# byronknoll/gmix

Measured on AMD Instinct MI355X. Metric: mixer bits/sec (synthetic 256-input mixer streams, forward+update), higher is better.
Workload: dtype f32; 1 GPU; configs[1]: synthetic 256-input 1-layer mixer (1 mixer, 2^16-row gate table), random logits, forward+update; n_inputs=256, mixers=1/0/0, streams_per_gpu=4096, total_bits=5452595200, parallelism=streams sharded over 1 GPU(s), no collective on the data path

## Files before the change

gmix_amd/csrc/gmx_capi.cpp:

```cpp
#include <hip/hip_runtime.h>
#include <math.h>
#include <stddef.h>
#include <stdio.h>
#include <stdlib.h>
#include <string.h>
#include <time.h>

#include <algorithm>
#include <cmath>
#include <atomic>
#include <map>
#include <new>
#include <string>
#include <vector>

#include "../../include/gmxmix.h"
#include "../../include/gmxmix_lstm_group.h"
#include "../../include/gmxmix_decoder.h"
#include "../../include/gmxmix_lstm_shape.h"
#include "../../include/gmxmix_encoder.h"
#include "../../include/gmxmix_analysis.h"
#include "../../include/gmxmix_ppmd.h"
#include "gmx_buildhash.h"
#include "gmx_internal.h"
// ... 1088 lines not shown
  a.seed = seed ? seed : 0x9E3779B97F4A7C15ull;
  a.n = t.n;
  a.n_pad = t.n_pad;
  a.m = t.m;
  a.mask_words = t.mask_words;
  a.n_streams = b->S;
  a.restart = restart ? 1 : 0;
  a.ctx_mode = ctx_mode;
  a.bit_mode = bit_mode;
  a.ctx_mod = ctx_mod;
  a.zero_mod = zero_mod;
  HIPCHK(gmx_launch_synth_kernel(&a, b->g->stream));
  return batch_note_device_use(b);
}

extern "C" int gmx_group_run(gmx_group* g, gmx_batch* b, uint64_t n_bits, int learn, float* kernel_ms) {
  if (!g || !b || b->g != g || b->S != g->S || n_bits > b->max_bits) return GMX_ERR_INVALID;
  HIPCHK(hipSetDevice(g->device));
  int rc = sessions_close(g, false);
  if (rc) return rc;
  std::fill(g->fwd_done.begin(), g->fwd_done.end(), 0);
  return launch_run(g, b, 0, 0, g->S, n_bits, GMX_MODE_PREDICT | (learn ? GMX_MODE_LEARN : 0u),
                    kernel_ms);
}

extern "C" int gmx_group_run_ragged(gmx_group* g, gmx_batch* b, const uint64_t* n_bits, int learn) {
  if (!g || !b || b->g != g || b->S != g->S || !n_bits) return GMX_ERR_INVALID;
  uint64_t maxn = 0;
  bool same = true;
  for (int s = 0; s < g->S; ++s) {
    if (n_bits[s] > b->max_bits) return GMX_ERR_INVALID;
    maxn = std::max(maxn, n_bits[s]);
    same = same && n_bits[s] == n_bits[0];
  }
  HIPCHK(hipSetDevice(g->device));
  int rc = sessions_close(g, false);
  if (rc) return rc;
  std::fill(g->fwd_done.begin(), g->fwd_done.end(), 0);
  const unsigned mode = GMX_MODE_PREDICT | (learn ? GMX_MODE_LEARN : 0u);
  if (same) return launch_run(g, b, 0, 0, g->S, maxn, mode, nullptr);
  const GmxKernelKind kind = kernel_for(g, mode);
  static const bool split = getenv("GMX_RAGGED_SPLIT") != nullptr;
  if (!split && (kind == GMX_K_STOCK || kind == GMX_K_BANK || kind == GMX_K_PAIR)) return launch_run(g, b, 0, 0, g->S, maxn, mode, nullptr, n_bits);
  for (int s0 = 0; s0 < g->S;) {
    int s1 = s0 + 1;
    while (s1 < g->S && n_bits[s1] == n_bits[s0]) ++s1;
    rc = launch_run(g, b, s0, s0, s1 - s0, n_bits[s0], mode, nullptr);
    if (rc) return rc;
    s0 = s1;
  }
  return GMX_OK;
}

static int ensure_one(gmx_group* g) {
  if (g->one) return GMX_OK;
  int rc = batch_alloc(&g->one, g, g->S, 1, GMX_BATCH_OUTPUTS | GMX_BATCH_MASK);
  if (rc) return rc;
  if (!gmx_batch_predictions(g->one) || !gmx_batch_active_mask(g->one) || !gmx_batch_contexts(g->one) ||
      !gmx_batch_bits(g->one) || !gmx_batch_p(g->one) || !gmx_batch_outputs(g->one))
    return GMX_ERR_NOMEM;
  return GMX_OK;
}

extern "C" int gmx_bank_forward(gmx_group* g, int stream, const float* predictions,
                                const int32_t* active_models, int n_active, const uint32_t* contexts,
                                float* p_final, float* out_all) {
  if (!g || stream < 0 || stream >= g->S || !predictions || !contexts) return GMX_ERR_INVALID;
  if (n_active > 0 && !active_models) return GMX_ERR_INVALID;
  HIPCHK(hipSetDevice(g->device));
  int rc;
  if (g->use_sessions && group_is_stock(g)) {
    rc = session_forward(g, stream, predictions, active_models, n_active, contexts, p_final, out_all);
    if (rc == GMX_OK) g->fwd_done[stream] = 2;
    if (rc != GMX_ERR_STATE) return rc;
  }
  rc = sessions_close(g, true);
  if (rc) return rc;
  rc = ensure_one(g);
  if (rc) return rc;
  gmx_batch* b = g->one;
  const GmxTopoDev& t = g->topo;
  const size_t s = (size_t)stream;
  HIPCHK(hipStreamSynchronize(g->stream));
  float* hp = b->h_pred + s * t.n_pad;
  uint32_t* hm = b->h_mask + s * t.mask_words;
  uint32_t* hc = b->h_ctx + s * t.m;
  memcpy(hp, predictions, t.n * sizeof(float));
  for (int i = t.n; i < t.n_pad; ++i) hp[i] = 0.f;
  if (n_active < 0) {
    for (int w = 0; w < t.mask_words; ++w) hm[w] = 0xffffffffu;
  } else {
    for (int w = 0; w < t.mask_words; ++w) hm[w] = 0;
    for (int i = 0; i < n_active; ++i) {
      int idx = active_models[i];
      if (idx < 0 || idx >= t.n) return GMX_ERR_INVALID;
      hm[idx >> 5] |= 1u << (idx & 31);
    }
  }
  memcpy(hc, contexts, t.m * sizeof(uint32_t));
  HIPCHK(hipMemcpyAsync(b->d_pred + s * t.n_pad, hp, t.n_pad * 4, hipMemcpyHostToDevice, g->stream));
  HIPCHK(hipMemcpyAsync(b->d_mask + s * t.mask_words, hm, t.mask_words * 4, hipMemcpyHostToDevice,
                        g->stream));
  HIPCHK(hipMemcpyAsync(b->d_ctx + s * t.m, hc, t.m * 4, hipMemcpyHostToDevice, g->stream));
  rc = launch_run(g, b, stream, stream, 1, 1, GMX_MODE_PREDICT | GMX_MODE_LATCH, nullptr);
  if (rc) return rc;
  HIPCHK(hipMemcpyAsync(b->h_p + s, b->d_p + s, 4, hipMemcpyDeviceToHost, g->stream));
  if (out_all)
    HIPCHK(hipMemcpyAsync(b->h_out + s * t.m, b->d_out + s * t.m, t.m * 4, hipMemcpyDeviceToHost,
                          g->stream));
  HIPCHK(hipStreamSynchronize(g->stream));
  if (p_final) *p_final = b->h_p[s];
  if (out_all) memcpy(out_all, b->h_out + s * t.m, t.m * sizeof(float));
  g->fwd_done[stream] = 1;
  return GMX_OK;
}

extern "C" int gmx_bank_learn(gmx_group* g, int stream, int bit) {
  if (!g || stream < 0 || stream >= g->S || (bit != 0 && bit != 1)) return GMX_ERR_INVALID;
  if (!g->fwd_done[stream]) return GMX_ERR_STATE;
  HIPCHK(hipSetDevice(g->device));
  if (g->fwd_done[stream] == 2) {
    int rcs = session_learn(g, stream, bit);
    if (rcs == GMX_OK) g->fwd_done[stream] = 0;
    return rcs;
  }
  if (!g->one) return GMX_ERR_STATE;
  gmx_batch* b = g->one;
  HIPCHK(hipStreamSynchronize(g->stream));
  b->h_bits[stream] = (uint8_t)bit;
  HIPCHK(hipMemcpyAsync(b->d_bits + stream, b->h_bits + stream, 1, hipMemcpyHostToDevice, g->stream));
  int rc = launch_run(g, b, stream, stream, 1, 1, GMX_MODE_LEARN, nullptr);
  if (rc) return rc;
  HIPCHK(hipStreamSynchronize(g->stream));
  g->fwd_done[stream] = 0;
  return GMX_OK;
}

#include "gmx_lockstep.inc"

static int fetch_bank(gmx_group* g, int stream, std::vector<uint8_t>& img) {
  img.resize(g->topo.bank_bytes);
  HIPCHK(hipSetDevice(g->device));
  int rc = sessions_close(g, true);
  if (rc) return rc;
  HIPCHK(hipStreamSynchronize(g->stream));
  HIPCHK(hipMemcpy(img.data(), g->banks + (size_t)stream * g->topo.bank_bytes, img.size(),
                   hipMemcpyDeviceToHost));
  return GMX_OK;
}

extern "C" int gmx_bank_export(gmx_group* g, int stream, void* long_buf, size_t* long_bytes,
                               void* short_buf, size_t* short_bytes) {
  if (!g || stream < 0 || stream >= g->S || !long_bytes || !short_bytes) return GMX_ERR_INVALID;
  const GmxTopoDev& t = g->topo;
  std::vector<uint8_t> img;
  int rc = fetch_bank(g, stream, img);
  if (rc) return rc;
  const size_t need_short = (size_t)t.m * 24;
  size_t need_long = 0;
  for (int j = 0; j < t.m; ++j) {
    need_long += 8;
    for (uint32_t r = 0; r < t.mx[j].table_size; ++r)
      if (*GMX_RS_PTR(img.data(), t.mx[j], r)) need_long += 12 + 4 * (size_t)t.mx[j].weight_size;
  }
  const bool fits = long_buf && short_buf && *long_bytes >= need_long && *short_bytes >= need_short;
  *long_bytes = need_long;
  *short_bytes = need_short;
  if (!long_buf && !short_buf) return GMX_OK;
  if (!fits) return GMX_ERR_INVALID;
  memcpy(short_buf, img.data() + t.scal_off, need_short);
  uint8_t* o = (uint8_t*)long_buf;
  for (int j = 0; j < t.m; ++j) {
    const GmxMixerDev& x = t.mx[j];
    const float* w = (const float*)(img.data() + x.w_off);
    uint32_t cnt = 0;
    for (uint32_t r = 0; r < x.table_size; ++r)
      if (*GMX_RS_PTR(img.data(), x, r)) ++cnt;
    uint32_t input_size = cnt ? x.weight_size : 0;
    memcpy(o, &cnt, 4);
    memcpy(o + 4, &input_size, 4);
    o += 8;
    for (uint32_t r = 0; r < x.table_size; ++r) {
      const uint64_t steps = *GMX_RS_PTR(img.data(), x, r);
      if (!steps) continue;
      memcpy(o, &r, 4);
      memcpy(o + 4, &steps, 8);
      memcpy(o + 12, w + (size_t)r * x.stride, 4 * (size_t)x.weight_size);
      o += 12 + 4 * (size_t)x.weight_size;
    }
  }
  return GMX_OK;
}

extern "C" int gmx_bank_import(gmx_group* g, int stream, const void* long_buf, size_t long_bytes,
                               const void* short_buf, size_t short_bytes) {
  if (!g || stream < 0 || stream >= g->S || !long_buf || !short_buf) return GMX_ERR_INVALID;
  const GmxTopoDev& t = g->topo;
  if (short_bytes != (size_t)t.m * 24) return GMX_ERR_FORMAT;
  std::vector<uint8_t> img(t.bank_bytes, 0);
  memcpy(img.data() + t.scal_off, short_buf, short_bytes);
  const uint64_t* sc = (const uint64_t*)(img.data() + t.scal_off);
  for (int j = 1; j < t.m; ++j)
    if (sc[3 * j] != sc[0]) return GMX_ERR_FORMAT;
  const uint8_t* p = (const uint8_t*)long_buf;
  const uint8_t* end = p + long_bytes;
  for (int j = 0; j < t.m; ++j) {
    const GmxMixerDev& x = t.mx[j];
    if (end - p < 8) return GMX_ERR_FORMAT;
    uint32_t cnt, input_size;
    memcpy(&cnt, p, 4);
    memcpy(&input_size, p + 4, 4);
    p += 8;
    if (cnt > x.table_size || (cnt && input_size != x.weight_size)) return GMX_ERR_FORMAT;
    float* w = (float*)(img.data() + x.w_off);
    for (uint32_t i = 0; i < cnt; ++i) {
      if ((size_t)(end - p) < 12 + 4 * (size_t)input_size) return GMX_ERR_FORMAT;
      uint32_t r;
      memcpy(&r, p, 4);
      if (r >= x.table_size) return GMX_ERR_FORMAT;
      uint64_t* const rs = GMX_RS_PTR(img.data(), x, r);
      memcpy(rs, p + 4, 8);
      if (*rs == 0) return GMX_ERR_FORMAT;
      memcpy(w + (size_t)r * x.stride, p + 12, 4 * (size_t)input_size);
      p += 12 + 4 * (size_t)input_size;
    }
  }
  if (p != end) return GMX_ERR_FORMAT;
  HIPCHK(hipSetDevice(g->device));
  int rc = sessions_close(g, true);
  if (rc) return rc;
  if (stream < (int)g->sessions.size() && g->sessions[stream]) g->sessions[stream]->fwd_live = false;
  HIPCHK(hipStreamSynchronize(g->stream));
  HIPCHK(hipMemcpy(g->banks + (size_t)stream * t.bank_bytes, img.data(), img.size(),
                   hipMemcpyHostToDevice));
  g->steps[stream] = sc[0];
  g->fwd_done[stream] = 0;
  for (gmx_lockstep* ls : g->locksteps) ls->predicted = false;
  return GMX_OK;
}

extern "C" int gmx_bank_copy(gmx_group* dst, int dst_stream, gmx_group* src, int src_stream) {
  if (!dst || !src || dst_stream < 0 || dst_stream >= dst->S || src_stream < 0 || src_stream >= src->S)
    return GMX_ERR_INVALID;
  const GmxTopoDev &a = dst->topo, &b = src->topo;
  if (a.m != b.m || a.n != b.n || a.n_skip != b.n_skip || a.bank_bytes != b.bank_bytes)
    return GMX_ERR_INVALID;
  for (int j = 0; j < a.m; ++j)
    if (a.mx[j].table_size != b.mx[j].table_size || a.mx[j].weight_size != b.mx[j].weight_size ||
        a.mx[j].layer != b.mx[j].layer)
      return GMX_ERR_INVALID;
  HIPCHK(hipSetDevice(src->device));
  int rc = sessions_close(src, true);
  if (rc) return rc;
  HIPCHK(hipStreamSynchronize(src->stream));
  HIPCHK(hipSetDevice(dst->device));
  rc = sessions_close(dst, true);
  if (rc) return rc;
  if (dst_stream < (int)dst->sessions.size() && dst->sessions[dst_stream])
    dst->sessions[dst_stream]->fwd_live = false;
  HIPCHK(hipStreamSynchronize(dst->stream));
  HIPCHK(hipMemcpy(dst->banks + (size_t)dst_stream * a.bank_bytes,
                   src->banks + (size_t)src_stream * b.bank_bytes, a.bank_bytes,
                   hipMemcpyDeviceToDevice));
  dst->steps[dst_stream] = src->steps[src_stream];
  dst->fwd_done[dst_stream] = 0;
  for (gmx_lockstep* ls : dst->locksteps) ls->predicted = false;
  return GMX_OK;
}

#include "gmx_ckpt.inc"

extern "C" int gmx_bank_memory_usage(gmx_group* g, int stream, int mixer, uint64_t* bytes) {
  if (!g || stream < 0 || stream >= g->S || mixer < 0 || mixer >= g->topo.m || !bytes)
    return GMX_ERR_INVALID;
  HIPCHK(hipSetDevice(g->device));
  int rc = sessions_close(g, true);
  if (rc) return rc;
  HIPCHK(hipStreamSynchronize(g->stream));
  uint64_t sc[3];
  HIPCHK(hipMemcpy(sc, g->banks + (size_t)stream * g->topo.bank_bytes + g->topo.scal_off + 24u * mixer,
                   24, hipMemcpyDeviceToHost));
  const GmxMixerDev& x = g->topo.mx[mixer];
  *bytes = 29 + sc[2] * (uint64_t)(x.weight_size * 4 + 12) + 8ull * x.table_size;
  return GMX_OK;
}


#include "gmx_indirect.inc"
#include "gmx_ind_ckpt.inc"
#include "gmx_lstm_any.inc"
#include "gmx_lstm.inc"
#include "gmx_lstm_ckpt.inc"
#include "gmx_match.inc"
#include "gmx_match_ckpt.inc"
#include "gmx_ctx.inc"
#include "gmx_ctx_ckpt.inc"
#include "gmx_chainstep.inc"
#include "gmx_coder.inc"
#include "gmx_encoder.inc"
#include "gmx_analysis.inc"
#include "gmx_ppmd.inc"

extern "C" int gmx_debug_single_variant(gmx_group* g, int lanes_per_stream) {
  if (!g || (lanes_per_stream != 0 && lanes_per_stream != 16 && lanes_per_stream != 32 &&
             lanes_per_stream != 64 && lanes_per_stream != 165 && lanes_per_stream != 325))
    return GMX_ERR_INVALID;
  g->single_variant = lanes_per_stream;
  return GMX_OK;
}

extern "C" int gmx_debug_stock_pairs(gmx_group* g, int on) {
  if (!g) return GMX_ERR_INVALID;
  g->stock_pairs = on != 0;
  return GMX_OK;
}

extern "C" int gmx_debug_decay_on_host(gmx_group* g, int on) {
  if (!g) return GMX_ERR_INVALID;
  g->decay_on_host = on != 0;
  return GMX_OK;
}

extern "C" int gmx_debug_decay_table(gmx_group* g, const uint64_t* steps0, int U, uint64_t T, float* out,
                                     uint32_t* n_unsettled) {
  if (!g || !steps0 || U < 1 || T < 1 || !out) return GMX_ERR_INVALID;
  HIPCHK(hipSetDevice(g->device));
  if (!g->copy_stream) HIPCHK(sibling_stream_create(&g->copy_stream, g->stream));
  gmx_group::DecaySlot tmp;
  std::map<uint64_t, uint32_t> uniq;
  std::vector<uint32_t> row(U);
  for (int u = 0; u < U; ++u) {
    auto it = uniq.find(steps0[u]);
    if (it == uniq.end()) it = uniq.emplace(steps0[u], (uint32_t)uniq.size()).first;
    row[u] = it->second;
  }
  HIPCHK(hipMalloc((void**)&tmp.dev, uniq.size() * T * sizeof(float)));
  int rc = decay_table_on_device(g, tmp, uniq, T);
  if (rc == GMX_OK) {
    if (n_unsettled) *n_unsettled = tmp.amb_host[0];
    std::vector<float> h(uniq.size() * T);
    hipError_t e = hipMemcpyAsync(h.data(), tmp.dev, h.size() * sizeof(float), hipMemcpyDeviceToHost, g->copy_stream);
    if (e == hipSuccess) e = hipStreamSynchronize(g->copy_stream);
    if (e != hipSuccess) rc = hip_fail(e, "gmx_debug_decay_table copy");
    else
      for (int u = 0; u < U; ++u) memcpy(out + (size_t)u * T, h.data() + (size_t)row[u] * T, T * sizeof(float));
  }
  void* dv[] = {tmp.dev, tmp.st_dev, tmp.amb_dev};
  for (void* p : dv)
    if (p) (void)hipFree(p);
  void* hv[] = {tmp.st_host, tmp.amb_host, tmp.patch_host};
  for (void* p : hv)
    if (p) (void)hipHostFree(p);
  return rc;
}

extern "C" int gmx_topology_register_rows_eligible(const gmx_topology* topo) {
  GmxTopoDev td;
  if (build_topology(topo, &td) != GMX_OK) return GMX_ERR_INVALID;
  return topo_register_rows_eligible(td) ? 1 : 0;
}

extern "C" int gmx_group_set_register_rows(gmx_group* g, int on) {
  if (!g || !topo_register_rows_eligible(g->topo)) return GMX_ERR_INVALID;
  g->register_rows = on != 0;
  return GMX_OK;
}

extern "C" int gmx_debug_force_general(gmx_group* g, int on) {
  if (!g) return GMX_ERR_INVALID;
  g->force_general = on != 0;
  return GMX_OK;
}

extern "C" int gmx_debug_kernel_kind(gmx_group* g, unsigned mode) {
  if (!g) return GMX_ERR_INVALID;
  const GmxKernelKind kind = kernel_for(g, mode);
  if (kind != GMX_K_BANK) return (int)kind;
  const GmxTopoDev& t = g->topo;
  return (int)kind + 4 * gmx_bank_kernel_build(t.l0, t.l1, t.n_skip, t.has_final, t.mx[t.l0 - 1].stride);
}

extern "C" int gmx_debug_stock_staged(gmx_group* g, int mode) {
  if (!g || mode < -1 || mode > 1) return GMX_ERR_INVALID;
  g->stock_staged = mode;
  return GMX_OK;
}

extern "C" int gmx_debug_stock_exact(gmx_group* g, int on) {
  if (!g) return GMX_ERR_INVALID;
  int rc = sessions_close(g, true);
  if (rc) return rc;
  g->stock_exact = on != 0;
  return GMX_OK;
}

extern "C" int gmx_debug_use_sessions(gmx_group* g, int on) {
  if (!g) return GMX_ERR_INVALID;
  int rc = sessions_close(g, true);
  if (rc) return rc;
  for (GmxSession* se : g->sessions)
    if (se && se->fwd_live) return GMX_ERR_STATE;
  g->use_sessions = on != 0;
  return GMX_OK;
}

extern "C" int gmx_debug_open_sessions(void) { return g_open_sessions.load(); }

extern "C" int gmx_debug_mailbox_on_device(gmx_group* g, int on, int stream, int* active) {
  if (!g) return GMX_ERR_INVALID;
  if (active) {
    GmxSession* se = (stream >= 0 && stream < (int)g->sessions.size()) ? g->sessions[stream] : nullptr;
    *active = (se && se->mc_on_device) ? 1 : 0;
  }
  if ((on != 0) == g->mailbox_on_device) return GMX_OK;
  int rc = sessions_close(g, true);
  if (rc) return rc;
  for (GmxSession* se : g->sessions)
    if (se && se->fwd_live) return GMX_ERR_STATE;
  sessions_free(g);
  g->mailbox_on_device = on != 0;
  return GMX_OK;
}

extern "C" int gmx_debug_per_bit_latency(gmx_group* g, int stream, int n, int ctx_hold, double* us_per_bit) {
  if (!g || n <= 0 || ctx_hold <= 0 || !us_per_bit) return GMX_ERR_INVALID;
  const GmxTopoDev& t = g->topo;
  std::vector<float> pred(t.n);
  std::vector<uint32_t> ctx(t.m, 0);
  uint64_t x = 0x9E3779B97F4A7C15ull;
  auto rnd = [&x]() { x ^= x << 13; x ^= x >> 7; x ^= x << 17; return x; };
  timespec a, b;
  clock_gettime(CLOCK_MONOTONIC, &a);
  for (int i = 0; i < n; ++i) {
    for (int k = 0; k < t.n; ++k) pred[k] = (float)((int64_t)(rnd() >> 40) - (1 << 23)) * (1.0f / (1 << 21));
    if (i % ctx_hold == 0)
      for (int k = 0; k < t.m; ++k) ctx[k] = (uint32_t)rnd();
    float p;
    int rc = gmx_bank_forward(g, stream, pred.data(), nullptr, -1, ctx.data(), &p, nullptr);
    if (rc) return rc;
    rc = gmx_bank_learn(g, stream, p > 0.5f ? 1 : 0);
    if (rc) return rc;
  }
  int rc = gmx_group_sync(g);
  if (rc) return rc;
  clock_gettime(CLOCK_MONOTONIC, &b);
  *us_per_bit = ((b.tv_sec - a.tv_sec) * 1e6 + (b.tv_nsec - a.tv_nsec) * 1e-3) / n;
  return GMX_OK;
}

static int stream_with_cu_mask(hipStream_t* st, const uint32_t* mask, int n_words) {
  hipStream_t fresh = nullptr;
  if (n_words > 0)
    HIPCHK(hipExtStreamCreateWithCUMask(&fresh, (uint32_t)n_words, mask));
  else if (*st)
    HIPCHK(sibling_stream_create(&fresh, *st));
  else
    HIPCHK(hipStreamCreateWithFlags(&fresh, hipStreamNonBlocking));
  if (*st) {
    (void)hipStreamSynchronize(*st);
    (void)hipStreamDestroy(*st);
  }
  *st = fresh;
  return GMX_OK;
}
extern "C" int gmx_group_set_cu_mask(gmx_group* g, const uint32_t* mask, int n_words) {
  if (!g || n_words < 0 || (n_words > 0 && !mask)) return GMX_ERR_INVALID;
  HIPCHK(hipSetDevice(g->device));
  int rc = sessions_close(g, false);
  if (rc) return rc;
  if (!g->locksteps.empty()) return GMX_ERR_STATE;
  return stream_with_cu_mask(&g->stream, mask, n_words);
}
extern "C" int gmx_indirect_set_cu_mask(gmx_indirect* ib, const uint32_t* mask, int n_words) {
  if (!ib || n_words < 0 || (n_words > 0 && !mask)) return GMX_ERR_INVALID;
  HIPCHK(hipSetDevice(ib->device));
  {
    int rcs = ind_sessions_close(ib);
    if (rcs) return rcs;
  }
  return stream_with_cu_mask(&ib->stream, mask, n_words);
}

extern "C" int gmx_debug_indirect_use_sessions(gmx_indirect* ib, int on) {
  if (!ib) return GMX_ERR_INVALID;
  HIPCHK(hipSetDevice(ib->device));
  int rc = ind_sessions_close(ib);
  if (rc) return rc;
  ib->use_sessions = on != 0;
  return GMX_OK;
}

static int chain_check_inputs(const gmx_indirect* ib, const GmxTopoDev& t, const int32_t* active_models, int n_active,
                              uint32_t* own) {
  if ((n_active > 0 && !active_models) || n_active > t.n) return GMX_ERR_INVALID;
  for (int i = 0; i < n_active; ++i)
    if (active_models[i] < 0 || active_models[i] >= t.n) return GMX_ERR_INVALID;
  for (int i = 0; i < ib->dev.k; ++i) {
    const int a = ib->dev.m[i].slot_a, b = ib->dev.m[i].slot_b;
    if (a < 0 || a >= t.n || b < 0 || b >= t.n) return GMX_ERR_INVALID;
    own[a >> 5] |= 1u << (a & 31);
    own[b >> 5] |= 1u << (b & 31);
  }
  return GMX_OK;
}

static void chain_put_indirect(const gmx_indirect* ib, const float* ipd, const uint8_t* iad, float* pred, uint32_t* mask) {
  for (int i = 0; i < ib->dev.k; ++i) {
    const int sl[2] = {ib->dev.m[i].slot_a, ib->dev.m[i].slot_b};
    for (int h = 0; h < 2; ++h) {
      pred[sl[h]] = ipd[2 * i + h];
      if (iad[2 * i + h]) mask[sl[h] >> 5] = mask[sl[h] >> 5] | (1u << (sl[h] & 31));
    }
  }
}

struct GmxChainMatch {
  gmx_match* mb;
  const uint32_t* ctx;
  float* predictions;
  uint8_t* active;
  uint32_t* longest_match;
};
static const int kChainNoSlot = 1;

struct GmxChainCtx {
  gmx_ctx* cb;
  uint32_t* values;
  bool want_values;
  uint32_t* bit_context;
};
static void chain_ctx_merge(const gmx_ctx* cb, int base, int n, const uint32_t* vals, const uint32_t* own, uint32_t* out) {
  for (int c = 0; c < n; ++c) {
    const int32_t rt = cb->routes[base + c];
    out[c] = rt >= 0 ? vals[rt] : (own ? own[c] : 0u);
  }
}

static int chain_forward_sessions(gmx_indirect* ib, gmx_group* g, int stream, const uint32_t* ind_contexts,
                                  uint32_t bit_context, const float* predictions, const int32_t* active_models,
                                  int n_active, const uint32_t* contexts, const uint32_t* own, float* p_final,
                                  float* out_all, float* ipd, uint8_t* iad, const GmxChainMatch* m,
                                  const GmxChainCtx* cx = nullptr) {
  gmx_match* const mb = m ? m->mb : nullptr;
  gmx_ctx* const cb = cx ? cx->cb : nullptr;
  GmxIndCtxCmd ccmd = {0, nullptr, nullptr};
  if (cx) {
    if (hipStreamQuery(cb->stream) != hipSuccess) HIPCHK(hipStreamSynchronize(cb->stream));
    (void)hipGetLastError();
    ccmd.what = GMX_STEP_PREDICT | (cx->want_values ? GMX_CTX_WAVE_VALUES : 0u) |
                (cb->wave_fresh[stream] ? 0u : GMX_CTX_WAVE_RELOAD);
    if (cb->noted[stream]) ccmd.what |= GMX_STEP_LEARN | ((uint32_t)(cb->noted[stream] - 1) << GMX_CTX_WAVE_BIT_SHIFT);
    ccmd.values = cx->values;
    ccmd.bit_context = cx->bit_context;
  }
  GmxIndMatchCmd mcmd;
  if (m) {
    if (hipStreamQuery(mb->stream) != hipSuccess) HIPCHK(hipStreamSynchronize(mb->stream));
    (void)hipGetLastError();
    const int noted = mb->noted[stream];
    mcmd = {m->ctx, kMatchStepPredict | kMatchStepTakeCtx, m->predictions, m->active, m->longest_match};
    if (noted) mcmd.what |= kMatchStepLearn | ((uint32_t)(noted - 1) << GMX_IND_MB_MATCH_BIT_SHIFT);
  }
  int rc = session_forward_prepare(g, stream, predictions, active_models, n_active, contexts, own);
  if (rc) return rc == GMX_ERR_STATE ? kChainNoSlot : rc;
  GmxSession* se = g->sessions[stream];
  rc = ind_session_forward(ib, stream, ind_contexts, bit_context, ipd, iad, se->word, se->slot, se->mc,
                           m ? &mcmd : nullptr, cx ? &ccmd : nullptr);
  bool ctx_by_launch = false;
  if (rc == GMX_OK) {
    ib->fwd_done[stream] = 2;
    if (cx) {
      if (cb->noted[stream]) {
        cb->noted[stream] = 0;
        cb->n_noted -= 1;
      }
      cb->outstanding[stream] = 1;
      cb->wave_fresh[stream] = 1;
      bit_context = *cx->bit_context;
    }
    if (m) {
      mb->noted[stream] = 0;
      mb->fwd_done[stream] = 2;
      mb->fwd_bc[stream] = bit_context;
    }
  } else {
    if (rc == GMX_ERR_STATE) {
      uint32_t icm[GMX_IND_MAX_MODELS], mcm[GMX_MATCH_MAX_MODELS];
      const uint32_t* ic = ind_contexts;
      const uint32_t* mc = m ? m->ctx : nullptr;
      rc = GMX_OK;
      if (cx) {
        rc = ctx_forward_launch(cb, stream, cx->values, cx->bit_context);
        if (rc == GMX_OK) {
          ctx_by_launch = true;
          bit_context = *cx->bit_context;
          chain_ctx_merge(cb, GMX_CTX_WAVE_ROUTE_IND, ib->dev.k, cx->values, ind_contexts, icm);
          ic = icm;
          if (m) {
            chain_ctx_merge(cb, GMX_CTX_WAVE_ROUTE_MATCH, mb->dev.k, cx->values, m->ctx, mcm);
            mc = mcm;
          }
        }
      }
      if (rc == GMX_OK && m) rc = match_flush_noted(mb, stream);
      if (m && rc == GMX_OK)
        rc = match_forward_launch(mb, stream, mc, bit_context, m->predictions, m->active, m->longest_match);
      if (rc == GMX_OK) rc = gmx_indirect_forward(ib, stream, ic, bit_context, ipd, iad);
    }
    if (rc != GMX_OK) {
// ... 292 lines not shown
```

gmix_amd/csrc/gmx_single.hip:

```cpp
#include <hip/hip_runtime.h>
#include <stdint.h>

#include "gmx_internal.h"
#include "gmx_math.h"

typedef float gmx_f4 __attribute__((ext_vector_type(4)));

template <int OFF>
__device__ __forceinline__ void gmx_ld16(gmx_f4& d, const float* p) {
  asm volatile("global_load_dwordx4 %0, %1, off offset:%2 nt" : "=v"(d) : "v"(p), "n"(OFF) : "memory");
}
__device__ __forceinline__ void gmx_ld8(uint64_t& d, const uint64_t* p) {
  asm volatile("global_load_dwordx2 %0, %1, off" : "=v"(d) : "v"(p) : "memory");
}
__device__ __forceinline__ void gmx_ld4(uint32_t& d, const void* p) {
  asm volatile("global_load_dword %0, %1, off" : "=v"(d) : "v"(p) : "memory");
}
__device__ __forceinline__ void gmx_ld1(uint32_t& d, const uint8_t* p) {
  asm volatile("global_load_ubyte %0, %1, off" : "=v"(d) : "v"(p) : "memory");
}
template <int OFF>
__device__ __forceinline__ void gmx_st16(float* p, const gmx_f4& v) {
  asm volatile("global_store_dwordx4 %0, %1, off offset:%2 nt" : : "v"(p), "v"(v), "n"(OFF) : "memory");
}
__device__ __forceinline__ void gmx_st8(uint64_t* p, uint64_t v) {
  asm volatile("global_store_dwordx2 %0, %1, off" : : "v"(p), "v"(v) : "memory");
}
__device__ __forceinline__ void gmx_st4(float* p, float v) {
  asm volatile("global_store_dword %0, %1, off" : : "v"(p), "v"(v) : "memory");
}

template <int K>
struct GmxSlot {
  gmx_f4 w[K];
  gmx_f4 x[K];
  uint32_t mk[K];
  uint64_t rs;
  uint32_t row;
  uint32_t bit;
  uint32_t dec;
};

template <int N>
__device__ __forceinline__ void gmx_wait_slot(GmxSlot<1>& a) {
  asm volatile("s_waitcnt vmcnt(%c5)"
               : "+v"(a.w[0]), "+v"(a.x[0]), "+v"(a.rs), "+v"(a.bit), "+v"(a.dec)
               : "n"(N));
}
template <int N>
__device__ __forceinline__ void gmx_wait_slot(GmxSlot<2>& a) {
  asm volatile("s_waitcnt vmcnt(%c7)"
               : "+v"(a.w[0]), "+v"(a.w[1]), "+v"(a.x[0]), "+v"(a.x[1]), "+v"(a.rs), "+v"(a.bit),
                 "+v"(a.dec)
               : "n"(N));
}
template <int N>
__device__ __forceinline__ void gmx_wait_slot(GmxSlot<4>& a) {
  asm volatile("s_waitcnt vmcnt(%c11)"
               : "+v"(a.w[0]), "+v"(a.w[1]), "+v"(a.w[2]), "+v"(a.w[3]), "+v"(a.x[0]), "+v"(a.x[1]),
                 "+v"(a.x[2]), "+v"(a.x[3]), "+v"(a.rs), "+v"(a.bit), "+v"(a.dec)
               : "n"(N));
}
template <int K>
__device__ __forceinline__ void gmx_pin_mask(GmxSlot<K>& a) {
  if (K == 1) asm volatile("" : "+v"(a.mk[0]));
  if (K == 2) asm volatile("" : "+v"(a.mk[0]), "+v"(a.mk[1 % K]));
  if (K == 4) asm volatile("" : "+v"(a.mk[0]), "+v"(a.mk[1 % K]), "+v"(a.mk[2 % K]), "+v"(a.mk[3 % K]));
}
__device__ __forceinline__ void gmx_pin(uint64_t& rs, uint32_t& bit, uint32_t& dec, uint32_t& cq) {
  asm volatile("" : "+v"(rs), "+v"(bit), "+v"(dec), "+v"(cq));
}

template <int LPS>
__device__ __forceinline__ float gmx_handoff(float acc, int i, bool first_pass, int lane) {
  const int a = __float_as_int(acc);
  if (LPS == 64)
    return __int_as_float(__builtin_amdgcn_update_dpp(0, a, 0x13C, 0xf, 0xf, false));
  if (LPS == 16)
    return __int_as_float(__builtin_amdgcn_update_dpp(0, a, 0x121, 0xf, 0xf, false));
  if (i == 16)
    return __int_as_float(__builtin_amdgcn_update_dpp(a, a, 0x142, 0xa, 0xf, false));
  if (i == 0 && !first_pass)
    return __shfl(acc, (lane & 32) | 31);
  return __int_as_float(__builtin_amdgcn_update_dpp(0, a, 0x121, 0xf, 0xf, false));
}

template <int K, int LPS>
__device__ __forceinline__ float gmx_chain_piece(const GmxSlot<K>& c, int q, float acc, int lane) {
  const float px = c.x[q].x * c.w[q].x, py = c.x[q].y * c.w[q].y;
  const float pz = c.x[q].z * c.w[q].z, pw = c.x[q].w * c.w[q].w;
#pragma unroll
  for (int i = 0; i < LPS; ++i) {
    acc = gmx_handoff<LPS>(acc, i, q == 0, lane) + px;
    acc = acc + py;
    acc = acc + pz;
    acc = acc + pw;
  }
  return acc;
}
template <int K, int LPS>
__device__ __forceinline__ float gmx_chain(const GmxSlot<K>& c, int lane) {
  float acc = 0.f;
#pragma unroll
  for (int q = 0; q < K; ++q) acc = gmx_chain_piece<K, LPS>(c, q, acc, lane);
  return acc;
}

template <int LPS, int K, int NSLOT, bool FULL, bool WANT_OUT, bool LEARN, bool HAS_MASK>
__global__ void __launch_bounds__(64)
gmx_single_kernel(const GmxTopoDev* __restrict__ tp, const GmxRunArgs a) {
  constexpr int G = 64 / LPS;
  constexpr int CH = 4 * LPS;
  constexpr int VM_PER_BIT = 1 + (WANT_OUT ? 1 : 0) + (LEARN ? K + 1 : 0) + 2 * K + 3 + (HAS_MASK ? K : 0) + 1;
  constexpr int VM_WAIT = 1 + (NSLOT - 2) * VM_PER_BIT;
  static_assert(VM_WAIT <= 63, "vmcnt is a 6-bit counter");
  static_assert(CH * 4 * (K - 1) < 4096, "immediate offset of global_load is 12 bits");
  const int lane = threadIdx.x;
  const int g = lane / LPS, l = lane % LPS;
  const int li = (int)blockIdx.x * G + g;
  __shared__ uint64_t s_tab[32];
  if (lane < 32) s_tab[lane] = gmx_exp2f_tab[lane];
  if (li >= a.n_streams) return;
  const int rec = a.rec_base + li;
  const int s = a.stream_base + li;
  const uint64_t T = a.T;
  if (T == 0) return;

  const int N = tp->n, NPAD = tp->n_pad;
  const uint32_t stride = FULL ? (uint32_t)(CH * K) : tp->mx[0].stride;
  const uint32_t table = tp->mx[0].table_size;
  const float lr = tp->mx[0].lr;
  uint8_t* const bank = a.banks + (uint64_t)s * tp->bank_bytes;
  float* const wtab = (float*)(bank + tp->mx[0].w_off);
  uint64_t* const rstab = (uint64_t*)(bank + tp->mx[0].rs_off);
  uint64_t* const scal = (uint64_t*)(bank + tp->scal_off);

  const uint64_t RS = a.rec_stride;
  const uint32_t xstride = FULL ? (uint32_t)(CH * K) : (uint32_t)NPAD;
  const float* const pred_s = a.pred + (uint64_t)rec * RS * xstride;
  const uint32_t* const ctx_s = a.ctx + (uint64_t)rec * RS;
  const uint8_t* const bits_s = a.bits + (uint64_t)rec * RS;
  const float* const dec_s = a.decay + (uint64_t)a.decay_idx[li] * T;
  const int MW = tp->mask_words;
  const uint32_t* const mask_s = HAS_MASK ? a.mask + (uint64_t)rec * RS * MW : nullptr;
  float* const p_s = a.p_out + (uint64_t)rec * RS;
  float* const oa_s = WANT_OUT ? a.out_all + (uint64_t)rec * RS : nullptr;

  uint64_t steps = scal[0], max_steps = scal[1], seen_cnt = scal[2];

  GmxSlot<K> sl[NSLOT];
  uint32_t ctxq[NSLOT];

  auto issue = [&](GmxSlot<K>& d, uint32_t ctx, uint64_t tb) {
    const uint64_t tt = tb < T ? tb : T - 1;
    d.row = ctx % table;
    const float* wr = wtab + (uint64_t)d.row * stride + 4 * l;
    const float* xr = pred_s + tt * (uint64_t)xstride + 4 * l;
    if (FULL) {
      gmx_ld16<0>(d.w[0], wr);
      if (K > 1) gmx_ld16<CH * 4>(d.w[1 % K], wr);
      if (K > 2) gmx_ld16<CH * 8>(d.w[2 % K], wr);
      if (K > 3) gmx_ld16<CH * 12>(d.w[3 % K], wr);
      gmx_ld16<0>(d.x[0], xr);
      if (K > 1) gmx_ld16<CH * 4>(d.x[1 % K], xr);
      if (K > 2) gmx_ld16<CH * 8>(d.x[2 % K], xr);
      if (K > 3) gmx_ld16<CH * 12>(d.x[3 % K], xr);
    } else {
#pragma unroll
      for (int k = 0; k < K; ++k) {
        const int e = CH * k + 4 * l;
        gmx_ld16<0>(d.w[k], (uint32_t)e < stride ? wr + CH * k : wr - 4 * l);
      }
#pragma unroll
      for (int k = 0; k < K; ++k) {
        const int e = CH * k + 4 * l;
        gmx_ld16<0>(d.x[k], e < NPAD ? xr + CH * k : xr - 4 * l);
      }
    }
    if (HAS_MASK) {
#pragma unroll
      for (int k = 0; k < K; ++k) {
        const int e = CH * k + 4 * l;
        gmx_ld4(d.mk[k], mask_s + tt * (uint64_t)MW + (e < NPAD ? (e >> 5) : 0));
      }
    }
    gmx_ld8(d.rs, rstab + d.row);
    gmx_ld1(d.bit, bits_s + tt);
    gmx_ld4(d.dec, dec_s + tt);
  };
  auto mask_inputs = [&](GmxSlot<K>& d) {
    if (!HAS_MASK) return;
#pragma unroll
    for (int k = 0; k < K; ++k) {
      const uint32_t b = d.mk[k] >> ((uint32_t)(CH * k + 4 * l) & 31u);
      d.x[k].x = (b & 1u) ? d.x[k].x : 0.f;
      d.x[k].y = (b & 2u) ? d.x[k].y : 0.f;
      d.x[k].z = (b & 4u) ? d.x[k].z : 0.f;
      d.x[k].w = (b & 8u) ? d.x[k].w : 0.f;
    }
  };
  auto trim = [&](GmxSlot<K>& d) {
    if (FULL) return;
#pragma unroll
    for (int k = 0; k < K; ++k) {
      const int e = CH * k + 4 * l;
      const bool wok = (uint32_t)e < stride;
      d.w[k].x = wok ? d.w[k].x : 0.f;
      d.w[k].y = wok ? d.w[k].y : 0.f;
      d.w[k].z = wok ? d.w[k].z : 0.f;
      d.w[k].w = wok ? d.w[k].w : 0.f;
      d.x[k].x = (e + 0 < N) ? d.x[k].x : 0.f;
      d.x[k].y = (e + 1 < N) ? d.x[k].y : 0.f;
      d.x[k].z = (e + 2 < N) ? d.x[k].z : 0.f;
      d.x[k].w = (e + 3 < N) ? d.x[k].w : 0.f;
    }
  };

#pragma unroll
  for (int k = 0; k < NSLOT; ++k) {
    const uint64_t tb = (uint64_t)k < T ? (uint64_t)k : T - 1;
    ctxq[k] = ctx_s[tb];
  }
#pragma unroll
  for (int k = 0; k < NSLOT; ++k) {
    issue(sl[k], ctxq[k], (uint64_t)k);
    const uint64_t tb = (uint64_t)(k + NSLOT) < T ? (uint64_t)(k + NSLOT) : T - 1;
    gmx_ld4(ctxq[k], ctx_s + tb);
  }
#pragma unroll
  for (int k = 0; k < NSLOT; ++k) {
    gmx_wait_slot<0>(sl[k]);
    if (HAS_MASK) gmx_pin_mask(sl[k]);
    gmx_pin(sl[k].rs, sl[k].bit, sl[k].dec, ctxq[k]);
  }
  trim(sl[0]);
  mask_inputs(sl[0]);
  float acc_cur = gmx_chain<K, LPS>(sl[0], lane);

  for (uint64_t t0 = 0; t0 < T; t0 += NSLOT) {
#pragma unroll
    for (int k = 0; k < NSLOT; ++k) {
      const uint64_t t = t0 + k;
      if (t >= T) break;
      GmxSlot<K>& c = sl[k];
      GmxSlot<K>& nx = sl[(k + 1) % NSLOT];
      gmx_wait_slot<VM_WAIT>(nx);
      if (HAS_MASK) gmx_pin_mask(nx);
      gmx_pin(c.rs, c.bit, c.dec, ctxq[k]);
      trim(nx);
      mask_inputs(nx);
      float acc_nxt = gmx_chain_piece<K, LPS>(nx, 0, 0.f, lane);
      float out = __shfl(acc_cur, lane | (LPS - 1));
      const bool seen = c.rs != 0;
      out = seen ? out : 0.f;
      const float pl = gmx_logistic_tab(out, s_tab);
      const float prob = gmx_clamp_prob(pl);
      gmx_st4(p_s + t, prob);
      if (WANT_OUT) gmx_st4(oa_s + t, out);
      if (K > 1) acc_nxt = gmx_chain_piece<K, LPS>(nx, 1 % K, acc_nxt, lane);
      if (!LEARN) {
        if (K > 2) acc_nxt = gmx_chain_piece<K, LPS>(nx, 2 % K, acc_nxt, lane);
        if (K > 3) acc_nxt = gmx_chain_piece<K, LPS>(nx, 3 % K, acc_nxt, lane);
      } else {
        const double dd = (double)__uint_as_float(c.dec) * (1.5 - ((double)c.rs) / (double)max_steps);
        const float decay = (float)dd;
        const float upd = decay * lr * (pl - (float)c.bit);
        const uint64_t rs_new = c.rs + 1;
        ++steps;
        max_steps = rs_new > max_steps ? rs_new : max_steps;
        seen_cnt += (c.rs == 0) ? 1u : 0u;
        const float sc = ((rs_new & 1023u) == 0) ? (1.0f - 3.0e-6f) : 1.0f;
        if (K > 2) acc_nxt = gmx_chain_piece<K, LPS>(nx, 2 % K, acc_nxt, lane);
#pragma unroll
        for (int q = 0; q < K; ++q) {
          c.w[q].x = (c.w[q].x - upd * c.x[q].x) * sc;
          c.w[q].y = (c.w[q].y - upd * c.x[q].y) * sc;
          c.w[q].z = (c.w[q].z - upd * c.x[q].z) * sc;
          c.w[q].w = (c.w[q].w - upd * c.x[q].w) * sc;
        }
        float* wr = wtab + (uint64_t)c.row * stride + 4 * l;
        if (FULL) {
          gmx_st16<0>(wr, c.w[0]);
          if (K > 1) gmx_st16<CH * 4>(wr, c.w[1 % K]);
          if (K > 2) gmx_st16<CH * 8>(wr, c.w[2 % K]);
          if (K > 3) gmx_st16<CH * 12>(wr, c.w[3 % K]);
        } else {
#pragma unroll
          for (int q = 0; q < K; ++q)
            if ((uint32_t)(CH * q + 4 * l) < stride) gmx_st16<0>(wr + CH * q, c.w[q]);
        }
        gmx_st8(rstab + c.row, rs_new);
        if (K > 3) acc_nxt = gmx_chain_piece<K, LPS>(nx, 3 % K, acc_nxt, lane);
        bool hit[NSLOT];
        bool any_hit = false;
#pragma unroll
        for (int j = 1; j < NSLOT; ++j) {
          hit[j] = sl[(k + j) % NSLOT].row == c.row && (t + j) < T;
          any_hit |= hit[j];
        }
        if (__any(any_hit)) {
#pragma unroll
          for (int j = 2; j < NSLOT; ++j) gmx_wait_slot<0>(sl[(k + j) % NSLOT]);
#pragma unroll
          for (int j = 1; j < NSLOT; ++j) {
            GmxSlot<K>& o = sl[(k + j) % NSLOT];
            if (hit[j]) {
#pragma unroll
              for (int q = 0; q < K; ++q) o.w[q] = c.w[q];
              o.rs = rs_new;
            }
          }
          if (__any(hit[1])) acc_nxt = gmx_chain<K, LPS>(nx, lane);
        }
      }
      issue(c, ctxq[k], t + NSLOT);
      {
        const uint64_t tn = t + 2 * NSLOT;
        gmx_ld4(ctxq[k], ctx_s + (tn < T ? tn : T - 1));
      }
      acc_cur = acc_nxt;
    }
  }
  asm volatile("s_waitcnt vmcnt(0)" ::: "memory");
  if (LEARN) {
    scal[0] = steps;
    scal[1] = max_steps;
    scal[2] = seen_cnt;
  }
}

template <int LPS, int K, int NSLOT, bool FULL, bool HAS_MASK>
static hipError_t launch_kfm(const GmxTopoDev* tp_dev, const GmxRunArgs& a, hipStream_t stream) {
  constexpr int G = 64 / LPS;
  const dim3 grid((a.n_streams + G - 1) / G), block(64);
  const bool learn = (a.mode & GMX_MODE_LEARN) != 0;
  if (a.out_all) {
    if (learn)
      hipLaunchKernelGGL((gmx_single_kernel<LPS, K, NSLOT, FULL, true, true, HAS_MASK>), grid, block, 0, stream, tp_dev, a);
    else
      hipLaunchKernelGGL((gmx_single_kernel<LPS, K, NSLOT, FULL, true, false, HAS_MASK>), grid, block, 0, stream, tp_dev, a);
  } else {
    if (learn)
      hipLaunchKernelGGL((gmx_single_kernel<LPS, K, NSLOT, FULL, false, true, HAS_MASK>), grid, block, 0, stream, tp_dev, a);
    else
      hipLaunchKernelGGL((gmx_single_kernel<LPS, K, NSLOT, FULL, false, false, HAS_MASK>), grid, block, 0, stream, tp_dev, a);
  }
  return hipGetLastError();
}
template <int LPS, int K, int NSLOT, bool FULL>
static hipError_t launch_kf(const GmxTopoDev* tp_dev, const GmxRunArgs& a, hipStream_t stream) {
  constexpr int VM_M = 1 + 1 + (K + 1) + 2 * K + 3 + K + 1;
  constexpr int NS_M = (1 + (NSLOT - 2) * VM_M <= 63) ? NSLOT : NSLOT - 1;
  return a.mask ? launch_kfm<LPS, K, NS_M, FULL, true>(tp_dev, a, stream)
                : launch_kfm<LPS, K, NSLOT, FULL, false>(tp_dev, a, stream);
}

template <int LPS, int K, int NSLOT>
static hipError_t launch_k(const GmxTopoDev* tp_dev, const GmxRunArgs& a, bool full,
                           hipStream_t stream) {
  return full ? launch_kf<LPS, K, NSLOT, true>(tp_dev, a, stream)
              : launch_kf<LPS, K, NSLOT, false>(tp_dev, a, stream);
}

extern "C" hipError_t gmx_launch_single_kernel(const GmxTopoDev* tp_dev, const GmxRunArgs* args,
                                               int n_inputs, int variant, hipStream_t stream) {
  (void)hipGetLastError();
  const GmxRunArgs& a = *args;
  if (n_inputs <= 64) return launch_k<16, 1, 4>(tp_dev, a, n_inputs == 64, stream);
  if (n_inputs <= 128) {
    if (variant == 16) return launch_k<16, 2, 4>(tp_dev, a, n_inputs == 128, stream);
    return launch_k<32, 1, 6>(tp_dev, a, n_inputs == 128, stream);
  }
  const bool full = n_inputs == 256;
  if (variant == 165) return launch_k<16, 4, 5>(tp_dev, a, full, stream);
  if (variant == 325) return launch_k<32, 2, 5>(tp_dev, a, full, stream);
  if (variant == 64) return launch_k<64, 1, 6>(tp_dev, a, full, stream);
  if (variant == 32) return launch_k<32, 2, 4>(tp_dev, a, full, stream);
  return launch_k<16, 4, 4>(tp_dev, a, full, stream);
}
```

Before: 1.832 billion bits/s.

## Skip weight-row loads for untouched gate rows using prefetched row-state hint

Prefetches each upcoming row's state word one slot earlier and, when it is zero (row never trained), masks off the weight-row loads with exec and zero-fills the weights instead. A late check reloads the row if it was updated in the meantime. This cuts global memory traffic for fresh rows in the 2^16-row table, at the cost of an extra load per bit, a deeper context prefetch queue, and extra exec-mask and ballot instructions. It is on by default (variant below 1000) except for some K=4 configurations.

```diff
diff --git a/gmix_amd/csrc/gmx_capi.cpp b/gmix_amd/csrc/gmx_capi.cpp
--- a/gmix_amd/csrc/gmx_capi.cpp
+++ b/gmix_amd/csrc/gmx_capi.cpp
@@ -1414,9 +1414,8 @@
 #include "gmx_ppmd.inc"
 
 extern "C" int gmx_debug_single_variant(gmx_group* g, int lanes_per_stream) {
-  if (!g || (lanes_per_stream != 0 && lanes_per_stream != 16 && lanes_per_stream != 32 &&
-             lanes_per_stream != 64 && lanes_per_stream != 165 && lanes_per_stream != 325))
-    return GMX_ERR_INVALID;
+  const int m = lanes_per_stream >= 1000 ? lanes_per_stream - 1000 : lanes_per_stream;
+  if (!g || (m != 0 && m != 16 && m != 32 && m != 64 && m != 165 && m != 325)) return GMX_ERR_INVALID;
   g->single_variant = lanes_per_stream;
   return GMX_OK;
 }
diff --git a/gmix_amd/csrc/gmx_single.hip b/gmix_amd/csrc/gmx_single.hip
--- a/gmix_amd/csrc/gmx_single.hip
+++ b/gmix_amd/csrc/gmx_single.hip
@@ -18,6 +18,70 @@
 }
 __device__ __forceinline__ void gmx_ld1(uint32_t& d, const uint8_t* p) {
   asm volatile("global_load_ubyte %0, %1, off" : "=v"(d) : "v"(p) : "memory");
+}
+template <int CHB>
+__device__ __forceinline__ void gmx_ld16_live(gmx_f4& d0, const float* p, uint64_t live) {
+  uint64_t sv;
+  asm volatile("s_and_saveexec_b64 %1, %3\n\t"
+               "global_load_dwordx4 %0, %2, off nt\n\t"
+               "s_mov_b64 exec, %1"
+               : "=&v"(d0), "=&s"(sv) : "v"(p), "s"(live) : "memory", "scc");
+}
+template <int CHB>
+__device__ __forceinline__ void gmx_ld16_live(gmx_f4& d0, gmx_f4& d1, const float* p, uint64_t live) {
+  uint64_t sv;
+  asm volatile("s_and_saveexec_b64 %2, %4\n\t"
+               "global_load_dwordx4 %0, %3, off nt\n\t"
+               "global_load_dwordx4 %1, %3, off offset:%5 nt\n\t"
+               "s_mov_b64 exec, %2"
+               : "=&v"(d0), "=&v"(d1), "=&s"(sv) : "v"(p), "s"(live), "n"(CHB) : "memory", "scc");
+}
+template <int CHB>
+__device__ __forceinline__ void gmx_ld16_live(gmx_f4& d0, gmx_f4& d1, gmx_f4& d2, gmx_f4& d3, const float* p,
+                                              uint64_t live) {
+  uint64_t sv;
+  asm volatile("s_and_saveexec_b64 %4, %6\n\t"
+               "global_load_dwordx4 %0, %5, off nt\n\t"
+               "global_load_dwordx4 %1, %5, off offset:%7 nt\n\t"
+               "global_load_dwordx4 %2, %5, off offset:%8 nt\n\t"
+               "global_load_dwordx4 %3, %5, off offset:%9 nt\n\t"
+               "s_mov_b64 exec, %4"
+               : "=&v"(d0), "=&v"(d1), "=&v"(d2), "=&v"(d3), "=&s"(sv)
+               : "v"(p), "s"(live), "n"(CHB), "n"(2 * CHB), "n"(3 * CHB)
+               : "memory", "scc");
+}
+__device__ __forceinline__ void gmx_ld16_live_rw(gmx_f4& d, const float* p, uint64_t live) {
+  uint64_t sv;
+  asm volatile("s_and_saveexec_b64 %1, %3\n\t"
+               "global_load_dwordx4 %0, %2, off nt\n\t"
+               "s_mov_b64 exec, %1"
+               : "+v"(d), "=&s"(sv) : "v"(p), "s"(live) : "memory", "scc");
+}
+__device__ __forceinline__ void gmx_ld16_live_at(gmx_f4& d0, const float* p0, uint64_t live) {
+  gmx_ld16_live<0>(d0, p0, live);
+}
+__device__ __forceinline__ void gmx_ld16_live_at(gmx_f4& d0, gmx_f4& d1, const float* p0, const float* p1,
+                                                 uint64_t live) {
+  uint64_t sv;
+  asm volatile("s_and_saveexec_b64 %2, %5\n\t"
+               "global_load_dwordx4 %0, %3, off nt\n\t"
+               "global_load_dwordx4 %1, %4, off nt\n\t"
+               "s_mov_b64 exec, %2"
+               : "=&v"(d0), "=&v"(d1), "=&s"(sv) : "v"(p0), "v"(p1), "s"(live) : "memory", "scc");
+}
+__device__ __forceinline__ void gmx_ld16_live_at(gmx_f4& d0, gmx_f4& d1, gmx_f4& d2, gmx_f4& d3, const float* p0,
+                                                 const float* p1, const float* p2, const float* p3,
+                                                 uint64_t live) {
+  uint64_t sv;
+  asm volatile("s_and_saveexec_b64 %4, %9\n\t"
+               "global_load_dwordx4 %0, %5, off nt\n\t"
+               "global_load_dwordx4 %1, %6, off nt\n\t"
+               "global_load_dwordx4 %2, %7, off nt\n\t"
+               "global_load_dwordx4 %3, %8, off nt\n\t"
+               "s_mov_b64 exec, %4"
+               : "=&v"(d0), "=&v"(d1), "=&v"(d2), "=&v"(d3), "=&s"(sv)
+               : "v"(p0), "v"(p1), "v"(p2), "v"(p3), "s"(live)
+               : "memory", "scc");
 }
 template <int OFF>
 __device__ __forceinline__ void gmx_st16(float* p, const gmx_f4& v) {
@@ -39,6 +103,7 @@
   uint32_t row;
   uint32_t bit;
   uint32_t dec;
+  uint32_t skip;
 };
 
 template <int N>
@@ -69,6 +134,10 @@
 }
 __device__ __forceinline__ void gmx_pin(uint64_t& rs, uint32_t& bit, uint32_t& dec, uint32_t& cq) {
   asm volatile("" : "+v"(rs), "+v"(bit), "+v"(dec), "+v"(cq));
+}
+
+__device__ __forceinline__ void gmx_pin(uint64_t& rs, uint32_t& bit, uint32_t& dec, uint32_t& cq, uint64_t& pk) {
+  asm volatile("" : "+v"(rs), "+v"(bit), "+v"(dec), "+v"(cq), "+v"(pk));
 }
 
 template <int LPS>
@@ -106,13 +175,14 @@
   return acc;
 }
 
-template <int LPS, int K, int NSLOT, bool FULL, bool WANT_OUT, bool LEARN, bool HAS_MASK>
+template <int LPS, int K, int NSLOT, bool FULL, bool WANT_OUT, bool LEARN, bool HAS_MASK, bool HINT>
 __global__ void __launch_bounds__(64)
 gmx_single_kernel(const GmxTopoDev* __restrict__ tp, const GmxRunArgs a) {
   constexpr int G = 64 / LPS;
   constexpr int CH = 4 * LPS;
-  constexpr int VM_PER_BIT = 1 + (WANT_OUT ? 1 : 0) + (LEARN ? K + 1 : 0) + 2 * K + 3 + (HAS_MASK ? K : 0) + 1;
-  constexpr int VM_WAIT = 1 + (NSLOT - 2) * VM_PER_BIT;
+  constexpr int VM_PER_BIT = 1 + (WANT_OUT ? 1 : 0) + (LEARN ? K + 1 : 0) + 2 * K + 3 + (HAS_MASK ? K : 0) +
+                             (HINT ? 1 : 0) + 1;
+  constexpr int VM_WAIT = (HINT ? 2 : 1) + (NSLOT - 2) * VM_PER_BIT;
   static_assert(VM_WAIT <= 63, "vmcnt is a 6-bit counter");
   static_assert(CH * 4 * (K - 1) < 4096, "immediate offset of global_load is 12 bits");
   const int lane = threadIdx.x;
@@ -150,26 +220,48 @@
 
   GmxSlot<K> sl[NSLOT];
   uint32_t ctxq[NSLOT];
-
-  auto issue = [&](GmxSlot<K>& d, uint32_t ctx, uint64_t tb) {
+  uint32_t rowq[NSLOT];
+  uint64_t pkq[NSLOT];
+
+  auto issue = [&](GmxSlot<K>& d, uint32_t row, bool skip, uint64_t tb) {
     const uint64_t tt = tb < T ? tb : T - 1;
-    d.row = ctx % table;
+    d.row = row;
+    d.skip = skip ? 1u : 0u;
     const float* wr = wtab + (uint64_t)d.row * stride + 4 * l;
     const float* xr = pred_s + tt * (uint64_t)xstride + 4 * l;
+    if (HINT) {
+      const uint64_t live = __ballot(!skip);
+      if constexpr (FULL) {
+        if constexpr (K == 1) gmx_ld16_live<CH * 4>(d.w[0], wr, live);
+        if constexpr (K == 2) gmx_ld16_live<CH * 4>(d.w[0], d.w[1], wr, live);
+        if constexpr (K == 4) gmx_ld16_live<CH * 4>(d.w[0], d.w[1], d.w[2], d.w[3], wr, live);
+      } else {
+        const float* wk[K];
+#pragma unroll
+        for (int k = 0; k < K; ++k) wk[k] = (uint32_t)(CH * k + 4 * l) < stride ? wr + CH * k : wr - 4 * l;
+        if constexpr (K == 1) gmx_ld16_live_at(d.w[0], wk[0], live);
+        if constexpr (K == 2) gmx_ld16_live_at(d.w[0], d.w[1], wk[0], wk[1], live);
+        if constexpr (K == 4) gmx_ld16_live_at(d.w[0], d.w[1], d.w[2], d.w[3], wk[0], wk[1], wk[2], wk[3], live);
+      }
+    }
     if (FULL) {
-      gmx_ld16<0>(d.w[0], wr);
-      if (K > 1) gmx_ld16<CH * 4>(d.w[1 % K], wr);
-      if (K > 2) gmx_ld16<CH * 8>(d.w[2 % K], wr);
-      if (K > 3) gmx_ld16<CH * 12>(d.w[3 % K], wr);
+      if (!HINT) {
+        gmx_ld16<0>(d.w[0], wr);
+        if (K > 1) gmx_ld16<CH * 4>(d.w[1 % K], wr);
+        if (K > 2) gmx_ld16<CH * 8>(d.w[2 % K], wr);
+        if (K > 3) gmx_ld16<CH * 12>(d.w[3 % K], wr);
+      }
       gmx_ld16<0>(d.x[0], xr);
       if (K > 1) gmx_ld16<CH * 4>(d.x[1 % K], xr);
       if (K > 2) gmx_ld16<CH * 8>(d.x[2 % K], xr);
       if (K > 3) gmx_ld16<CH * 12>(d.x[3 % K], xr);
     } else {
-#pragma unroll
-      for (int k = 0; k < K; ++k) {
-        const int e = CH * k + 4 * l;
-        gmx_ld16<0>(d.w[k], (uint32_t)e < stride ? wr + CH * k : wr - 4 * l);
+      if (!HINT) {
+#pragma unroll
+        for (int k = 0; k < K; ++k) {
+          const int e = CH * k + 4 * l;
+          gmx_ld16<0>(d.w[k], (uint32_t)e < stride ? wr + CH * k : wr - 4 * l);
+        }
       }
 #pragma unroll
       for (int k = 0; k < K; ++k) {
@@ -216,22 +308,54 @@
     }
   };
 
+  auto unskip = [&](GmxSlot<K>& d, bool in_batch) {
+    if (!HINT) return;
+    const bool late = in_batch && d.skip != 0 && d.rs != 0;
+    if (__any(late)) {
+      const uint64_t lm = __ballot(late);
+      const float* wr = wtab + (uint64_t)d.row * stride + 4 * l;
+#pragma unroll
+      for (int k = 0; k < K; ++k)
+        gmx_ld16_live_rw(d.w[k], FULL || (uint32_t)(CH * k + 4 * l) < stride ? wr + CH * k : wr - 4 * l, lm);
+      gmx_wait_slot<0>(d);
+      d.skip = late ? 0u : d.skip;
+    }
+    const bool z = d.skip != 0;
+#pragma unroll
+    for (int k = 0; k < K; ++k) {
+      d.w[k].x = z ? 0.f : d.w[k].x;
+      d.w[k].y = z ? 0.f : d.w[k].y;
+      d.w[k].z = z ? 0.f : d.w[k].z;
+      d.w[k].w = z ? 0.f : d.w[k].w;
+    }
+    d.skip = 0;
+  };
+  const auto tclamp = [&](uint64_t tb) { return tb < T ? tb : T - 1; };
+
+  uint32_t row0[NSLOT];
 #pragma unroll
   for (int k = 0; k < NSLOT; ++k) {
-    const uint64_t tb = (uint64_t)k < T ? (uint64_t)k : T - 1;
-    ctxq[k] = ctx_s[tb];
+    row0[k] = ctx_s[tclamp(k)] % table;
+    if (HINT) rowq[k] = ctx_s[tclamp(k + NSLOT)] % table;
   }
 #pragma unroll
   for (int k = 0; k < NSLOT; ++k) {
-    issue(sl[k], ctxq[k], (uint64_t)k);
-    const uint64_t tb = (uint64_t)(k + NSLOT) < T ? (uint64_t)(k + NSLOT) : T - 1;
-    gmx_ld4(ctxq[k], ctx_s + tb);
+    issue(sl[k], row0[k], false, (uint64_t)k);
+    if (HINT) {
+      gmx_ld8(pkq[k], rstab + rowq[k]);
+      gmx_ld4(ctxq[k], ctx_s + tclamp(k + 2 * NSLOT));
+    } else {
+      gmx_ld4(ctxq[k], ctx_s + tclamp(k + NSLOT));
+    }
   }
 #pragma unroll
   for (int k = 0; k < NSLOT; ++k) {
     gmx_wait_slot<0>(sl[k]);
     if (HAS_MASK) gmx_pin_mask(sl[k]);
-    gmx_pin(sl[k].rs, sl[k].bit, sl[k].dec, ctxq[k]);
+    if (HINT)
+      gmx_pin(sl[k].rs, sl[k].bit, sl[k].dec, ctxq[k], pkq[k]);
+    else
+      gmx_pin(sl[k].rs, sl[k].bit, sl[k].dec, ctxq[k]);
   }
   trim(sl[0]);
   mask_inputs(sl[0]);
@@ -246,7 +370,11 @@
       GmxSlot<K>& nx = sl[(k + 1) % NSLOT];
       gmx_wait_slot<VM_WAIT>(nx);
       if (HAS_MASK) gmx_pin_mask(nx);
-      gmx_pin(c.rs, c.bit, c.dec, ctxq[k]);
+      if (HINT)
+        gmx_pin(c.rs, c.bit, c.dec, ctxq[k], pkq[k]);
+      else
+        gmx_pin(c.rs, c.bit, c.dec, ctxq[k]);
+      unskip(nx, t + 1 < T);
       trim(nx);
       mask_inputs(nx);
       float acc_nxt = gmx_chain_piece<K, LPS>(nx, 0, 0.f, lane);
@@ -308,15 +436,20 @@
 #pragma unroll
               for (int q = 0; q < K; ++q) o.w[q] = c.w[q];
               o.rs = rs_new;
+              o.skip = 0;
             }
           }
           if (__any(hit[1])) acc_nxt = gmx_chain<K, LPS>(nx, lane);
         }
       }
-      issue(c, ctxq[k], t + NSLOT);
-      {
-        const uint64_t tn = t + 2 * NSLOT;
-        gmx_ld4(ctxq[k], ctx_s + (tn < T ? tn : T - 1));
+      if (HINT) {
+        issue(c, rowq[k], pkq[k] == 0, t + NSLOT);
+        rowq[k] = ctxq[k] % table;
+        gmx_ld8(pkq[k], rstab + rowq[k]);
+        gmx_ld4(ctxq[k], ctx_s + tclamp(t + 3 * NSLOT));
+      } else {
+        issue(c, ctxq[k] % table, false, t + NSLOT);
+        gmx_ld4(ctxq[k], ctx_s + tclamp(t + 2 * NSLOT));
       }
       acc_cur = acc_nxt;
     }
@@ -329,52 +462,59 @@
   }
 }
 
-template <int LPS, int K, int NSLOT, bool FULL, bool HAS_MASK>
+template <int LPS, int K, int NSLOT, bool FULL, bool HAS_MASK, bool HINT>
 static hipError_t launch_kfm(const GmxTopoDev* tp_dev, const GmxRunArgs& a, hipStream_t stream) {
   constexpr int G = 64 / LPS;
   const dim3 grid((a.n_streams + G - 1) / G), block(64);
   const bool learn = (a.mode & GMX_MODE_LEARN) != 0;
   if (a.out_all) {
     if (learn)
-      hipLaunchKernelGGL((gmx_single_kernel<LPS, K, NSLOT, FULL, true, true, HAS_MASK>), grid, block, 0, stream, tp_dev, a);
+      hipLaunchKernelGGL((gmx_single_kernel<LPS, K, NSLOT, FULL, true, true, HAS_MASK, HINT>), grid, block, 0, stream, tp_dev, a);
     else
-      hipLaunchKernelGGL((gmx_single_kernel<LPS, K, NSLOT, FULL, true, false, HAS_MASK>), grid, block, 0, stream, tp_dev, a);
+      hipLaunchKernelGGL((gmx_single_kernel<LPS, K, NSLOT, FULL, true, false, HAS_MASK, HINT>), grid, block, 0, stream, tp_dev, a);
   } else {
     if (learn)
-      hipLaunchKernelGGL((gmx_single_kernel<LPS, K, NSLOT, FULL, false, true, HAS_MASK>), grid, block, 0, stream, tp_dev, a);
+      hipLaunchKernelGGL((gmx_single_kernel<LPS, K, NSLOT, FULL, false, true, HAS_MASK, HINT>), grid, block, 0, stream, tp_dev, a);
     else
-      hipLaunchKernelGGL((gmx_single_kernel<LPS, K, NSLOT, FULL, false, false, HAS_MASK>), grid, block, 0, stream, tp_dev, a);
+      hipLaunchKernelGGL((gmx_single_kernel<LPS, K, NSLOT, FULL, false, false, HAS_MASK, HINT>), grid, block, 0, stream, tp_dev, a);
   }
   return hipGetLastError();
 }
-template <int LPS, int K, int NSLOT, bool FULL>
+template <int LPS, int K, int NSLOT, bool FULL, bool HINT>
 static hipError_t launch_kf(const GmxTopoDev* tp_dev, const GmxRunArgs& a, hipStream_t stream) {
-  constexpr int VM_M = 1 + 1 + (K + 1) + 2 * K + 3 + K + 1;
-  constexpr int NS_M = (1 + (NSLOT - 2) * VM_M <= 63) ? NSLOT : NSLOT - 1;
-  return a.mask ? launch_kfm<LPS, K, NS_M, FULL, true>(tp_dev, a, stream)
-                : launch_kfm<LPS, K, NSLOT, FULL, false>(tp_dev, a, stream);
+  constexpr bool HINT_M = HINT && !(K == 4 && !FULL);
+  constexpr bool HINT_N = HINT && !(K == 4 && NSLOT == 5);
+  constexpr int VM_M = 1 + 1 + (K + 1) + 2 * K + 3 + K + (HINT_M ? 1 : 0) + 1;
+  constexpr int NS_M = ((HINT_M ? 2 : 1) + (NSLOT - 2) * VM_M <= 63) ? NSLOT : NSLOT - 1;
+  return a.mask ? launch_kfm<LPS, K, NS_M, FULL, true, HINT_M>(tp_dev, a, stream)
+                : launch_kfm<LPS, K, NSLOT, FULL, false, HINT_N>(tp_dev, a, stream);
 }
 
 template <int LPS, int K, int NSLOT>
-static hipError_t launch_k(const GmxTopoDev* tp_dev, const GmxRunArgs& a, bool full,
+static hipError_t launch_k(const GmxTopoDev* tp_dev, const GmxRunArgs& a, bool full, bool hint,
                            hipStream_t stream) {
-  return full ? launch_kf<LPS, K, NSLOT, true>(tp_dev, a, stream)
-              : launch_kf<LPS, K, NSLOT, false>(tp_dev, a, stream);
+  if (hint)
+    return full ? launch_kf<LPS, K, NSLOT, true, true>(tp_dev, a, stream)
+                : launch_kf<LPS, K, NSLOT, false, true>(tp_dev, a, stream);
+  return full ? launch_kf<LPS, K, NSLOT, true, false>(tp_dev, a, stream)
+              : launch_kf<LPS, K, NSLOT, false, false>(tp_dev, a, stream);
 }
 
 extern "C" hipError_t gmx_launch_single_kernel(const GmxTopoDev* tp_dev, const GmxRunArgs* args,
                                                int n_inputs, int variant, hipStream_t stream) {
   (void)hipGetLastError();
   const GmxRunArgs& a = *args;
-  if (n_inputs <= 64) return launch_k<16, 1, 4>(tp_dev, a, n_inputs == 64, stream);
+  const bool hint = variant < 1000;
+  variant %= 1000;
+  if (n_inputs <= 64) return launch_k<16, 1, 4>(tp_dev, a, n_inputs == 64, hint, stream);
   if (n_inputs <= 128) {
-    if (variant == 16) return launch_k<16, 2, 4>(tp_dev, a, n_inputs == 128, stream);
-    return launch_k<32, 1, 6>(tp_dev, a, n_inputs == 128, stream);
+    if (variant == 16) return launch_k<16, 2, 4>(tp_dev, a, n_inputs == 128, hint, stream);
+    return launch_k<32, 1, 6>(tp_dev, a, n_inputs == 128, hint, stream);
   }
   const bool full = n_inputs == 256;
-  if (variant == 165) return launch_k<16, 4, 5>(tp_dev, a, full, stream);
-  if (variant == 325) return launch_k<32, 2, 5>(tp_dev, a, full, stream);
-  if (variant == 64) return launch_k<64, 1, 6>(tp_dev, a, full, stream);
-  if (variant == 32) return launch_k<32, 2, 4>(tp_dev, a, full, stream);
-  return launch_k<16, 4, 4>(tp_dev, a, full, stream);
-}
+  if (variant == 165) return launch_k<16, 4, 5>(tp_dev, a, full, hint, stream);
+  if (variant == 325) return launch_k<32, 2, 5>(tp_dev, a, full, hint, stream);
+  if (variant == 64) return launch_k<64, 1, 6>(tp_dev, a, full, hint, stream);
+  if (variant == 32) return launch_k<32, 2, 4>(tp_dev, a, full, hint, stream);
+  return launch_k<16, 4, 4>(tp_dev, a, full, hint, stream);
+}
```

Result: no change. 1.837 billion bits/s, median of 6 (+0.3%).
